# backtato/ai-video-detector

Hardware: AMD Instinct MI355X
Metric: sampled frames/sec analysed (1080p30 60 s clip, 2 fps sampling) (higher is better)
Workload: dtype u8 pixels; f32/f64 Farneback (cv2's own types); 1 GPU; BASELINE.json configs[1]: 1080p30 60 s clip, 2 fps sampling, one clip per GPU per step; frames_per_clip=120, height=1080, width=1920, clips_in_flight_per_gpu=3, fb_mode=fast+rerun, fb_wide160=2, parallelism=single GPU, rccl_ranks_seen=1

## Files before the change

ai-video-detector_amd/csrc/avd_farneback.hip:

```cpp
#include "avd_internal.h"
#include "avd_fb_device.h"

#pragma clang fp contract(off)

namespace {

constexpr int S = AVD_SMALL;

template <int K>
struct PyrGeo {
    static constexpr int WL = S >> K;
    static constexpr int NC = K == 0 ? S : 2 * WL;
    static constexpr int OFF = K == 0 ? 0 : (1 << K) / 2 - 1;
    static constexpr int TR = K >= 2 ? 4 : 8;
    static constexpr int STEPS = K >= 2 ? 2 : 1, BAND = STEPS * TR;
    static constexpr int TILES = WL / BAND;
    static constexpr int KS = K == 3 ? 19 : (K == 2 ? 9 : 3), HALF = KS / 2;
    static constexpr int SROWS = K == 0 ? TR + 2 * HALF : ((TR - 1) << K) + 2 + 2 * HALF;
    static constexpr int NEW = K == 0 ? TR : TR << K, KEEP = SROWS - NEW;
    static constexpr int PADX = 12, PS = S + 2 * PADX;
    static constexpr int SRC_BYTES = SROWS * PS, LDS_BYTES = SRC_BYTES + SROWS * NC * 4;
    static constexpr int FILTERED_PCT = TILES * (SROWS + (STEPS - 1) * NEW) * 100 / S;
    static_assert(WL % BAND == 0 && (K == 0 || FILTERED_PCT <= 120), "whole bands; a source row is filtered at most 1.2 times per frame");
    static_assert(STEPS == 1 || (KEEP * NC <= 4 * 256 && SRC_BYTES % 16 == 0 && (NEW * NC) % 4 == 0 && (KEEP * NC) % 4 == 0),
                  "the rows a step takes over move as one 16-byte piece per lane");
};
constexpr int cmax(int a, int b) { return a > b ? a : b; }
constexpr int cgcd(int a, int b) { return b == 0 ? a : cgcd(b, a % b); }

template <int PR>
struct PyrWalk {
    static constexpr int PER = PR / cgcd(256, PR), SG = 256 / cgcd(256, PR);
    __device__ static __forceinline__ void first(int tid, int& r, int& c)
    {
        r = 0; c = tid;
#pragma unroll
        for (int q = 1; q * PR < 256; q++)
            if (tid >= q * PR) { r = q; c = tid - q * PR; }
    }
    __device__ static __forceinline__ void next(int& r, int& c)
    {
        r += 256 / PR; c += 256 % PR;
        if (c >= PR) { c -= PR; r++; }
    }
};
constexpr int kPyrLds = cmax(cmax(PyrGeo<3>::LDS_BYTES, PyrGeo<2>::LDS_BYTES), cmax(PyrGeo<1>::LDS_BYTES, PyrGeo<0>::LDS_BYTES));

typedef float pyr_f4 __attribute__((ext_vector_type(4)));
typedef float pyr_f2 __attribute__((ext_vector_type(2)));

template <bool MA>
__device__ __forceinline__ float pyr_mac(float a, float b, float c)
{
    if constexpr (MA) return __fadd_rn(__fmul_rn(a, b), c);
    else return __builtin_fmaf(a, b, c);
}

template <int K, bool MA = false, bool LERP = false>
__device__ __forceinline__ void pyramid_step(char* lds, const uint8_t* __restrict__ img, const float (&kw)[PyrGeo<K>::KS], float* __restrict__ out,
                                             int y_first, int rb, pyr_f4& kept, bool more, int* __restrict__ diffword)
{
    using G = PyrGeo<K>;
    constexpr int WL = G::WL, NC = G::NC, OFF = G::OFF, TR = G::TR, KS = G::KS, HALF = G::HALF, SROWS = G::SROWS;
    constexpr int PADX = G::PADX, PS = G::PS;
    uint8_t (*src)[PS] = reinterpret_cast<uint8_t (*)[PS]>(lds);
    float (*rowf)[NC] = reinterpret_cast<float (*)[NC]>(lds + G::SRC_BYTES);
    const int tid = threadIdx.x;
    const bool cmp = K == 1 && diffword != nullptr;
    static_assert(K != 1 || G::STEPS == 1, "the pair-identity word is formed by a tile that loads all its source rows in one step");
    static_assert(HALF + 1 < S, "a source row is reflected at most once");
    auto row_at = [&](int r) -> unsigned { const int y = y_first + r; return (unsigned)(y < 0 ? -y : (y >= S ? 2 * S - 2 - y : y)) * S; };
    constexpr int NLD = (SROWS * (S / 4) + 255) / 256, NBD = (SROWS * 2 * HALF + 255) / 256;
    const int nld = (SROWS - rb) * (S / 4), nbd = (SROWS - rb) * 2 * HALF;
    constexpr int NBATCH = 8;
    int differs = 0;
#pragma unroll
    for (int e0 = 0; e0 < NLD; e0 += NBATCH) {
        const bool last = e0 + NBATCH >= NLD;
        unsigned v[NBATCH], vn[K == 1 ? NBATCH : 1];
        uint8_t bv[NBD];
#pragma unroll
        for (int e = e0; e < NLD && e < e0 + NBATCH; e++) {
            const int it = tid + 256 * e, q = it / (S / 4), c4 = it - q * (S / 4);
            if (it >= nld) continue;
            const unsigned at = row_at(rb + q) + 4u * c4;
            v[e - e0] = *reinterpret_cast<const unsigned*>(img + at);
            if (K == 1 && cmp) vn[e - e0] = *reinterpret_cast<const unsigned*>(img + (at + AVD_NPIX));
        }
#pragma unroll
        for (int e = 0; e < NBD; e++) {
            const int it = tid + 256 * e, q = it / (2 * HALF), i = it - q * (2 * HALF);
            if (!last || it >= nbd) continue;
            bv[e] = img[row_at(rb + q) + (unsigned)(i < HALF ? 1 + i : S - 2 - (i - HALF))];
        }
#pragma unroll
        for (int e = e0; e < NLD && e < e0 + NBATCH; e++) {
            const int it = tid + 256 * e, q = it / (S / 4), c4 = it - q * (S / 4);
            if (it >= nld) continue;
            reinterpret_cast<unsigned*>(src[rb + q] + PADX)[c4] = v[e - e0];
            if (K == 1 && cmp) differs |= v[e - e0] != vn[e - e0];
        }
#pragma unroll
        for (int e = 0; e < NBD; e++) {
            const int it = tid + 256 * e, q = it / (2 * HALF), i = it - q * (2 * HALF);
            if (!last || it >= nbd) continue;
            src[rb + q][i < HALF ? PADX - 1 - i : PADX + S + (i - HALF)] = bv[e];
        }
        __builtin_amdgcn_sched_barrier(0);
    }
    if (K == 1 && cmp) {
        const int any = __syncthreads_or(differs);
        if (tid == 0) *diffword = any;
    } else
        __syncthreads();
    if (G::STEPS > 1 && rb && tid < G::KEEP * NC / 4) reinterpret_cast<pyr_f4*>(&rowf[0][0])[tid] = kept;
    if (KS == 3) {
        static_assert(KS != 3 || NC == S, "the 3-tap scales filter whole rows");
        using W = PyrWalk<S / 4>;
        const unsigned* wp0[W::PER]; pyr_f4* dst0[W::PER]; int r0[W::PER];
        {
            int r, c4;
            W::first(tid, r, c4);
#pragma unroll
            for (int i = 0; i < W::PER; i++) {
                r0[i] = r;
                wp0[i] = reinterpret_cast<const unsigned*>(src[r] + PADX + 4 * c4);
                dst0[i] = reinterpret_cast<pyr_f4*>(&rowf[r][4 * c4]);
                W::next(r, c4);
            }
        }
        for (int sb = rb; sb < SROWS; sb += W::SG) {
#pragma unroll
            for (int i = 0; i < W::PER; i++) {
                if (256 * i >= SROWS * (S / 4) || r0[i] + sb >= SROWS) continue;
                const unsigned* wp = wp0[i] + sb * (PS / 4);
                const unsigned pw = wp[-1], cwd = wp[0], nw = wp[1];
                const float b[6] = {(float)(pw >> 24), (float)(cwd & 0xFFu), (float)((cwd >> 8) & 0xFFu), (float)((cwd >> 16) & 0xFFu),
                                    (float)(cwd >> 24), (float)(nw & 0xFFu)};
                pyr_f4 o;
#pragma unroll
                for (int e = 0; e < 4; e++) o[e] = pyr_mac<MA>(b[e + 1], kw[1], (b[e] + b[e + 2]) * kw[0]);
                dst0[i][sb * (NC / 4)] = o;
            }
        }
    } else {
        static_assert(KS == 3 || (K >= 2 && NC == 2 * WL), "the long filters run at the decimated scales, where the columns are pairs");
        using W = PyrWalk<WL>;
        constexpr int B0 = PADX + OFF - HALF, SH = B0 & 3, NW = (SH + KS + 1 + 3) / 4;
        const unsigned* wp0[W::PER]; pyr_f2* dst0[W::PER]; int r0[W::PER];
        {
            int r, jp;
            W::first(tid, r, jp);
#pragma unroll
            for (int i = 0; i < W::PER; i++) {
                r0[i] = r;
                wp0[i] = reinterpret_cast<const unsigned*>(src[r] + (B0 & ~3) + (jp << K));
                dst0[i] = reinterpret_cast<pyr_f2*>(&rowf[r][2 * jp]);
                W::next(r, jp);
            }
        }
        for (int sb = rb; sb < SROWS; sb += W::SG) {
#pragma unroll
            for (int i = 0; i < W::PER; i++) {
                if (256 * i >= SROWS * WL || r0[i] + sb >= SROWS) continue;
                const unsigned* wp = wp0[i] + sb * (PS / 4);
                unsigned d[NW];
#pragma unroll
                for (int q = 0; q < NW; q++) d[q] = wp[q];
                float b[KS + 1];
#pragma unroll
                for (int q = 0; q <= KS; q++) b[q] = (float)((d[(SH + q) >> 2] >> (8 * ((SH + q) & 3))) & 0xFFu);
                float v0 = 0.f, v1 = 0.f;
#pragma unroll
                for (int q = 0; q < KS; q++) {
                    v0 = pyr_mac<MA>(b[q], kw[q], v0);
                    v1 = pyr_mac<MA>(b[q + 1], kw[q], v1);
                }
                dst0[i][sb * (NC / 2)] = pyr_f2{v0, v1};
            }
        }
    }
    __syncthreads();
    auto colf = [&](const float* c) {
        float sacc = pyr_mac<MA>(c[0], kw[HALF], 0.f);
#pragma unroll
        for (int k = 1; k <= HALF; k++) sacc = pyr_mac<MA>(c[k * NC] + c[-k * NC], kw[HALF + k], sacc);
        return sacc;
    };
    {
        using W = PyrWalk<WL>;
        int dyl, dx;
        W::first(tid, dyl, dx);
#pragma unroll
        for (int i = 0; i < W::PER; i++) {
            if (256 * i < TR * WL) {
                for (int y = dyl; y < TR; y += W::SG) {
                    float o;
                    if (K == 0) {
                        o = colf(&rowf[y + HALF][dx]);
                    } else {
                        const pyr_f2* c = reinterpret_cast<const pyr_f2*>(&rowf[y << K][2 * dx]);
                        float w[2][2 * HALF + 2];
#pragma unroll
                        for (int q = 0; q < 2 * HALF + 2; q++) {
                            const pyr_f2 v = c[q * (NC / 2)];
                            w[0][q] = v.x; w[1][q] = v.y;
                        }
                        float p[2][2];
#pragma unroll
                        for (int a = 0; a < 2; a++)
#pragma unroll
                            for (int e = 0; e < 2; e++) {
                                float sacc = pyr_mac<MA>(w[e][HALF + a], kw[HALF], 0.f);
#pragma unroll
                                for (int k = 1; k <= HALF; k++) sacc = pyr_mac<MA>(w[e][HALF + a + k] + w[e][HALF + a - k], kw[HALF + k], sacc);
                                p[a][e] = sacc;
                            }
                        if constexpr (LERP && K >= 2) {
                            const float h0 = p[0][0] + (p[0][1] - p[0][0]) * 0.5f, h1 = p[1][0] + (p[1][1] - p[1][0]) * 0.5f;
                            o = h0 + (h1 - h0) * 0.5f;
                        } else
                            o = ((p[0][0] + p[0][1]) + (p[1][0] + p[1][1])) * 0.25f;
                    }
                    out[y * WL + dx] = o;
                }
            }
            W::next(dyl, dx);
        }
    }
    if (G::STEPS > 1 && more && tid < G::KEEP * NC / 4) kept = reinterpret_cast<const pyr_f4*>(&rowf[G::NEW][0])[tid];
}

template <int K, bool MA = false, bool LERP = false>
__device__ __forceinline__ void pyramid_body(char* lds, int blk, const uint8_t* __restrict__ small, const FbConsts* __restrict__ C,
                                             float* __restrict__ I, int n = 0, int* __restrict__ pairdiff = nullptr)
{
    using G = PyrGeo<K>;
    constexpr int WL = G::WL;
    const int f = blk / G::TILES, t = blk - f * G::TILES;
    const int dy0 = t * G::BAND;
    const uint8_t* img = small + (int64_t)f * AVD_NPIX;
    float* out = I + ((int64_t)f * WL + dy0) * WL;
    int* diffword = K == 1 && pairdiff != nullptr && f + 1 < n ? pairdiff + blk : nullptr;
    float kw[G::KS];
#pragma unroll
    for (int q = 0; q < G::KS; q++) kw[q] = C->gk[K][q];
    const int y_first = (K == 0 ? dy0 : (dy0 << K) + G::OFF) - G::HALF;
    pyr_f4 kept = {0.f, 0.f, 0.f, 0.f};
    for (int step = 0; step < G::STEPS; step++)
        pyramid_step<K, MA, LERP>(lds, img, kw, out + step * G::TR * WL, y_first + step * G::NEW, step ? G::KEEP : 0, kept, step + 1 < G::STEPS, diffword);
}


template <bool MA, bool LERP>
__device__ __forceinline__ void pyramid_all(char* lds, const uint8_t* __restrict__ small, int n, const FbConsts* __restrict__ C,
                                            float* __restrict__ I0, float* __restrict__ I1, float* __restrict__ I2,
                                            float* __restrict__ I3, int* __restrict__ flags, int* __restrict__ pairdiff)
{
    static_assert(PyrGeo<1>::TILES == kPairDiffTiles, "avd_fbfast.hip reads one word per 160-px tile");
    if (flags && (int)(blockIdx.x * 256 + threadIdx.x) < n - 1) flags[blockIdx.x * 256 + threadIdx.x] = 0;
    const int n3 = n * PyrGeo<3>::TILES, n2 = n * PyrGeo<2>::TILES, n1 = n * PyrGeo<1>::TILES;
    int b = blockIdx.x;
    if (b < n3) { pyramid_body<3, MA, LERP>(lds, b, small, C, I3); return; }
    b -= n3;
    if (b < n2) { pyramid_body<2, MA, LERP>(lds, b, small, C, I2); return; }
    b -= n2;
    if (b < n1) { pyramid_body<1, MA, LERP>(lds, b, small, C, I1, n, pairdiff); return; }
    if (I0) pyramid_body<0, MA, LERP>(lds, b - n1, small, C, I0);
}

__global__ __launch_bounds__(256) void k_pyramid_all(const uint8_t* __restrict__ small, int n, const FbConsts* __restrict__ C,
                                                    float* __restrict__ I0, float* __restrict__ I1, float* __restrict__ I2,
                                                    float* __restrict__ I3, int* __restrict__ flags, int* __restrict__ pairdiff)
{
    __shared__ __align__(16) char lds[kPyrLds];
    pyramid_all<false, false>(lds, small, n, C, I0, I1, I2, I3, flags, pairdiff);
}

template <bool MA, bool LERP>
__global__ __launch_bounds__(256) void k_pyramid_model(const uint8_t* __restrict__ small, int n, const FbConsts* __restrict__ C,
                                                      float* __restrict__ I0, float* __restrict__ I1, float* __restrict__ I2,
                                                      float* __restrict__ I3, int* __restrict__ flags, int* __restrict__ pairdiff)
{
    __shared__ __align__(16) char lds[kPyrLds];
    pyramid_all<MA, LERP>(lds, small, n, C, I0, I1, I2, I3, flags, pairdiff);
}

struct PolyPtrs { const float* I[AVD_FB_LEVELS]; float* R[AVD_FB_LEVELS]; const uint8_t* small; };

constexpr int kPolyRows = 16;
constexpr int kPolyQuads = 4 * (S / 4 + 10);
static_assert(AVD_FB_LEVELS == 4, "three walking scales and the one-row form of the coarsest");
__host__ __device__ constexpr int poly_wgs(int k) { return k < AVD_FB_LEVELS - 1 ? (S >> k) / kPolyRows : S >> (2 * k); }

typedef float pf4 __attribute__((ext_vector_type(4)));
typedef float pf2 __attribute__((ext_vector_type(2)));

__device__ __forceinline__ void polyexp_put(pf4* __restrict__ rowq, int x, int w, float t0, float t1, float t2)
{
    const pf4 t = {t0, t1, t1, t2};
    rowq[x + 5] = t;
    if (x == 0)
        for (int q = 0; q < 5; q++) rowq[q] = t;
    if (x == w - 1)
        for (int q = 0; q < 5; q++) rowq[w + 5 + q] = t;
}

__device__ __forceinline__ void polyexp_hpass(const pf4* __restrict__ rq, const float (&g)[6], const float (&xg)[6], const double (&gd)[6],
                                              const double (&xxgd)[6], double ig11, double ig03, double ig33, double ig55, float* __restrict__ o)
{
    const pf4 c = rq[0];
    double b1 = (double)(c.x * g[0]), b2 = 0, b3 = (double)(c.y * g[0]), b4 = 0, b5 = (double)(c.w * g[0]), b6 = 0;
#pragma unroll
    for (int q = 1; q <= 5; q++) {
        const pf4 p = rq[q], m = rq[-q];
        const pf2 s01 = p.xy + m.xy, d01 = p.xy - m.xy, s12 = p.zw + m.zw;
        const pf2 dx = d01 * pf2{xg[q], xg[q]};
        const pf2 sg = s12 * pf2{g[q], g[q]};
        const double tg = (double)s01.x;
        b1 = __builtin_fma(tg, gd[q], b1);
        b4 = __builtin_fma(tg, xxgd[q], b4);
        b2 += (double)dx.x;
        b3 += (double)sg.x;
        b6 += (double)dx.y;
        b5 += (double)sg.y;
    }
    o[0] = (float)(b3 * ig11);
    o[1] = (float)(b2 * ig11);
    o[2] = (float)(b1 * ig03 + b5 * ig33);
    o[3] = (float)(b1 * ig03 + b4 * ig33);
    o[4] = (float)(b6 * ig55);
}

template <int K, bool FOLD>
__device__ __forceinline__ void polyexp_rows(const float* __restrict__ img, const uint8_t* __restrict__ small, float* __restrict__ out, int y0,
                                             const FbConsts* __restrict__ C, pf4 (*rowb)[kPolyQuads], float (*outb)[S * 5])
{
    static_assert(!FOLD || K == 0, "only the 320-px scale forms its own blur");
    constexpr int w = S >> K, h = w, R = 1 << K, STEPS = kPolyRows / R;
    static_assert(R * (w + 10) <= kPolyQuads && h % kPolyRows == 0 && kPolyRows % R == 0, "a step's R rows fit one LDS buffer; whole bands");
    const int tid = threadIdx.x;
    const int sr = K == 0 ? 0 : tid / w, x = tid - sr * w;
    const int yb = y0 + sr;
    const int xs = x - 1 < 0 ? 0 : (x - 1 > w - 4 ? w - 4 : x - 1);
    const int shl = ((x == 0 ? 1 : x - 1) - xs) * 8, shc = (x - xs) * 8, shr = ((x == w - 1 ? w - 2 : x + 1) - xs) * 8;
    const float kx0 = C->gk[0][0], kx1 = C->gk[0][1], kx2 = C->gk[0][2];
    struct __attribute__((packed, aligned(1))) U4 { unsigned v; };
    auto hb = [&](int srow) __attribute__((always_inline)) {
        const int sr = srow < 0 ? -srow : (srow > h - 1 ? 2 * (h - 1) - srow : srow);
        const unsigned wd = reinterpret_cast<const U4*>(small + sr * w + xs)->v;
        const float l = (float)((wd >> shl) & 0xFFu), c = (float)((wd >> shc) & 0xFFu), r = (float)((wd >> shr) & 0xFFu);
        return __builtin_fmaf(c, kx1, (l + r) * kx0);
    };
    float hm = 0.f, h0 = 0.f, hp = 0.f;
    int rcur = -1000;
    auto blurred = [&](int r) __attribute__((always_inline)) {
        if (r != rcur) {
            if (r == rcur + 1) { hm = h0; h0 = hp; hp = hb(r + 1); }
            else { hm = hb(r - 1); h0 = hb(r); hp = hb(r + 1); }
            rcur = r;
        }
        return __builtin_fmaf(hp + hm, kx2, __builtin_fmaf(h0, kx1, 0.f));
    };
    auto pixel = [&](int r) __attribute__((always_inline)) { return FOLD ? blurred(r) : img[r * w + x]; };
    typedef float f4 __attribute__((ext_vector_type(4)));
    typedef float f2 __attribute__((ext_vector_type(2)));
    float g[6], xg[6], xxg[6];
    double gd[6], xxgd[6];
#pragma unroll
    for (int q = 0; q <= 5; q++) { g[q] = C->g[5 + q]; xg[q] = C->xg[5 + q]; xxg[q] = C->xxg[5 + q]; gd[q] = C->gd[q]; xxgd[q] = C->xxgd[q]; }
    const double ig11 = C->ig11, ig03 = C->ig03, ig33 = C->ig33, ig55 = C->ig55;
    float win[11 + kPolyRows - R];
#pragma unroll
    for (int q = 0; q < 10; q++) win[q] = pixel(min(max(yb - 5 + q, 0), h - 1));
    pf4* rowq[2] = {rowb[0] + sr * (w + 10), rowb[1] + sr * (w + 10)};
#pragma unroll
    for (int i = 0; i < STEPS; i++) {
        const int par = i & 1, o = R * i;
#pragma unroll
        for (int j = o + 11 - R; j <= o + 10; j++)
            if (j >= 10) win[j] = pixel(min(yb - 5 + j, h - 1));
        {
            f2 t02 = f2{win[o + 5] * g[0], 0.f};
            float t1 = 0.f;
#pragma unroll
            for (int q = 1; q <= 5; q++) {
                const float a = win[o + 5 - q], bb = win[o + 5 + q];
                const float p = a + bb;
                t02 = t02 + f2{g[q], xxg[q]} * f2{p, p};
                t1 = t1 + xg[q] * (bb - a);
            }
            polyexp_put(rowq[par], x, w, t02.x, t1, t02.y);
        }
        __syncthreads();
        if (i > 0) {
            f4* dst = reinterpret_cast<f4*>(out + (int64_t)(y0 + o - R) * w * 5);
            const f4* srcv = reinterpret_cast<const f4*>(outb[par ^ 1]);
            __builtin_nontemporal_store(srcv[tid], dst + tid);
            if (tid < S * 5 / 4 - 320) __builtin_nontemporal_store(srcv[tid + 320], dst + tid + 320);
        }
        polyexp_hpass(rowq[par] + x + 5, g, xg, gd, xxgd, ig11, ig03, ig33, ig55, outb[par] + tid * 5);
    }
    __syncthreads();
    {
        f4* dst = reinterpret_cast<f4*>(out + (int64_t)(y0 + kPolyRows - R) * w * 5);
        const f4* srcv = reinterpret_cast<const f4*>(outb[(STEPS - 1) & 1]);
        __builtin_nontemporal_store(srcv[tid], dst + tid);
        if (tid < S * 5 / 4 - 320) __builtin_nontemporal_store(srcv[tid + 320], dst + tid + 320);
    }
}

__global__ __launch_bounds__(320) void k_polyexp_all(PolyPtrs P, int n, const FbConsts* __restrict__ C)
{
    __shared__ pf4 rowb[2][kPolyQuads];
    __shared__ __align__(16) float outbb[2][S * 5];
    pf4* row = rowb[0];
    static_assert(8 * (S / 8 + 10) <= 2 * kPolyQuads, "the eight sub-rows of the coarsest scale fit");
    float* outb = outbb[0];
    int b = (int)blockIdx.x, k = 0, wgs = 0;
    for (; k < AVD_FB_LEVELS; k++) {
        wgs = n * poly_wgs(k);
        const int cnt = ((wgs + 7) >> 3) << 3;
        if (b < cnt) break;
        b -= cnt;
    }
    if (k >= AVD_FB_LEVELS) return;
    const int per = (wgs + 7) >> 3, lid = (b & 7) * per + (b >> 3);
    if (lid >= wgs) return;
    const int w = S >> k, h = w;
    int f = 0;
#pragma unroll
    for (int kk = 0; kk < AVD_FB_LEVELS; kk++)
        if (k == kk) f = lid / poly_wgs(kk);
    const int t = lid - f * poly_wgs(k);
    float* R = P.R[k] + (int64_t)f * w * h * 5;
    if (k == 0) {
        if (P.small) polyexp_rows<0, true>(nullptr, P.small + (int64_t)f * S * S, R, t * kPolyRows, C, rowb, outbb);
        else polyexp_rows<0, false>(P.I[0] + (int64_t)f * S * S, nullptr, R, t * kPolyRows, C, rowb, outbb);
        return;
    }
    if (k == 1) { polyexp_rows<1, false>(P.I[1] + (int64_t)f * w * h, nullptr, R, t * kPolyRows, C, rowb, outbb); return; }
    if (k == 2) { polyexp_rows<2, false>(P.I[2] + (int64_t)f * w * h, nullptr, R, t * kPolyRows, C, rowb, outbb); return; }
    const int y0 = t << k;
    const int tid = threadIdx.x;
    const int sr = tid / w, x = tid - sr * w;
    const int y = y0 + sr;
    const float* img = P.I[k] + (int64_t)f * w * h;
    float g[6], xg[6], xxg[6];
    double gd[6], xxgd[6];
#pragma unroll
    for (int q = 0; q <= 5; q++) { g[q] = C->g[5 + q]; xg[q] = C->xg[5 + q]; xxg[q] = C->xxg[5 + q]; gd[q] = C->gd[q]; xxgd[q] = C->xxgd[q]; }
    pf4* rowq = row + sr * (w + 10);
    {
        float t0 = img[y * w + x] * g[0], t1 = 0.f, t2 = 0.f;
#pragma unroll
        for (int q = 1; q <= 5; q++) {
            const float a = img[max(y - q, 0) * w + x], bb = img[min(y + q, h - 1) * w + x];
            const float p = a + bb;
            t0 = t0 + g[q] * p;
            t1 = t1 + xg[q] * (bb - a);
            t2 = t2 + xxg[q] * p;
        }
        polyexp_put(rowq, x, w, t0, t1, t2);
    }
    __syncthreads();
    polyexp_hpass(rowq + x + 5, g, xg, gd, xxgd, C->ig11, C->ig03, C->ig33, C->ig55, outb + tid * 5);
    __syncthreads();
    typedef float f4 __attribute__((ext_vector_type(4)));
    f4* dst = reinterpret_cast<f4*>(R + (int64_t)y0 * w * 5);
    const f4* srcv = reinterpret_cast<const f4*>(outb);
    __builtin_nontemporal_store(srcv[tid], dst + tid);
    if (tid < S * 5 / 4 - 320) __builtin_nontemporal_store(srcv[tid + 320], dst + tid + 320);
}

template <int W, bool LERP = false>
__global__ __launch_bounds__(256) void k_flow_up(const float* __restrict__ prev, float* __restrict__ flow, int npairs, const int* __restrict__ plist)
{
    constexpr int H = W, PW = W / 2, PH = H / 2, Q = W / 4;
    const int gid = blockIdx.x * 256 + threadIdx.x;
    if (gid >= npairs * 2 * H * Q) return;
    const int q = gid % Q;
    const int dy = (gid / Q) % H;
    int pc = gid / (Q * H);
    if (plist) pc = plist[pc >> 1] * 2 + (pc & 1);
    const float* src = prev + (int64_t)pc * PW * PH;
    float fy = dy * 0.5f - 0.25f;
    const int sy = floor_f(fy);
    fy -= sy;
    const float* r0 = src + clampi(sy, 0, PH - 1) * PW;
    const float* r1 = src + clampi(sy + 1, 0, PH - 1) * PW;
    const float b0 = 1.f - fy, b1 = fy;
    float o[4];
#pragma unroll
    for (int i = 0; i < 4; i++) {
        const int dx = q * 4 + i;
        float fx = dx * 0.5f - 0.25f;
        int sx = floor_f(fx);
        fx -= sx;
        if (sx < 0) { fx = 0; sx = 0; }
        bool edge = false;
        if (sx + 1 >= PW) { edge = true; if (sx >= PW - 1) { fx = 0; sx = PW - 1; } }
        const int x1 = min(sx + 1, PW - 1);
        const float a0 = 1.f - fx, a1 = fx;
        float d0, d1;
        if (edge) { d0 = r0[sx] * 1.f; d1 = r1[sx] * 1.f; }
        else if constexpr (LERP) { d0 = r0[sx] + (r0[x1] - r0[sx]) * a1; d1 = r1[sx] + (r1[x1] - r1[sx]) * a1; }
        else { d0 = r0[sx] * a0 + r0[x1] * a1; d1 = r1[sx] * a0 + r1[x1] * a1; }
        if constexpr (LERP) o[i] = (d0 + (d1 - d0) * b1) * 2.f;
        else o[i] = (d0 * b0 + d1 * b1) * 2.f;
    }
    *reinterpret_cast<float4*>(flow + ((int64_t)pc * H + dy) * W + q * 4) = make_float4(o[0], o[1], o[2], o[3]);
}

constexpr int kChunk = 8192;
constexpr int kNChunk = (AVD_NPIX + kChunk - 1) / kChunk;

__device__ __forceinline__ float chunk_total(const float* part)
{
    float t = part[0];
#pragma unroll
    for (int i = 1; i < kNChunk; i++) t += part[i];
    return t;
}

__global__ __launch_bounds__(512) void k_stats_pair(const float* __restrict__ mag, float* __restrict__ stats, const int* __restrict__ plist)
{
    __shared__ float wpart[kNChunk][8];
    __shared__ float ctot[kNChunk];
    const int p = plist ? plist[blockIdx.x] : (int)blockIdx.x, tid = threadIdx.x;
    const int l = tid >> 3, wave = tid >> 6;
    const bool in_last = l < ((AVD_NPIX - (kNChunk - 1) * kChunk) >> 7);
    const float* src = mag + (int64_t)p * AVD_NPIX + l * 128 + (tid & 7);
    float v[kNChunk][16];
#pragma unroll
    for (int c = 0; c < kNChunk; c++)
#pragma unroll
        for (int k = 0; k < 16; k++) v[c][k] = (c < kNChunk - 1 || in_last) ? src[c * kChunk + 8 * k] : 0.f;
    float total[2];
#pragma unroll
    for (int pass = 0; pass < 2; pass++) {
#pragma unroll
        for (int c = 0; c < kNChunk; c++) {
            float r = v[c][0];
#pragma unroll
            for (int k = 1; k < 16; k++) r += v[c][k];
#pragma unroll
            for (int d = 1; d < 64; d <<= 1) r = r + __shfl_down(r, d);
            if ((tid & 63) == 0) wpart[c][wave] = r;
        }
        __syncthreads();
        if (tid < kNChunk) {
            const float* w = wpart[tid];
            ctot[tid] = tid < kNChunk - 1 ? ((w[0] + w[1]) + (w[2] + w[3])) + ((w[4] + w[5]) + (w[6] + w[7])) : (w[0] + w[1]) + (w[2] + w[3]);
        }
        __syncthreads();
        total[pass] = chunk_total(ctot);
        if (pass == 0) {
            const float mean32 = total[0] / (float)AVD_NPIX;
#pragma unroll
            for (int c = 0; c < kNChunk; c++)
#pragma unroll
                for (int k = 0; k < 16; k++) { const float d = v[c][k] - mean32; v[c][k] = d * d; }
            __syncthreads();
        }
    }
    if (tid == 0) {
        stats[2 * p] = (float)((double)total[0] / (double)AVD_NPIX);
        stats[2 * p + 1] = (float)((double)total[1] / (double)AVD_NPIX);
    }
}

__global__ void k_mag(const float* __restrict__ flow, float* __restrict__ mag, int64_t total4, const int* __restrict__ plist)
{
    const int64_t gid = (int64_t)blockIdx.x * 256 + threadIdx.x;
    if (gid >= total4) return;
    const int64_t ps = gid / (AVD_NPIX / 4), i = gid - ps * (AVD_NPIX / 4);
    const int64_t p = plist ? plist[ps] : ps;
    const float4 fx = reinterpret_cast<const float4*>(flow + p * 2 * AVD_NPIX)[i], fy = reinterpret_cast<const float4*>(flow + (p * 2 + 1) * AVD_NPIX)[i];
    float4 m;
    m.x = sqrtf(fx.x * fx.x + fy.x * fy.x);
    m.y = sqrtf(fx.y * fx.y + fy.y * fy.y);
    m.z = sqrtf(fx.z * fx.z + fy.z * fy.z);
    m.w = sqrtf(fx.w * fx.w + fy.w * fy.w);
    reinterpret_cast<float4*>(mag + p * AVD_NPIX)[i] = m;
}

__global__ void k_flow_interleave(const float* __restrict__ flow, float* __restrict__ out, int64_t total)
{
    const int64_t gid = (int64_t)blockIdx.x * 256 + threadIdx.x;
    if (gid >= total) return;
    const int64_t p = gid / AVD_NPIX, i = gid - p * AVD_NPIX;
    out[gid * 2] = flow[p * 2 * AVD_NPIX + i];
    out[gid * 2 + 1] = flow[(p * 2 + 1) * AVD_NPIX + i];
}

template <typename... A>
inline void launch1d(void (*k)(A...), int64_t items, int block, hipStream_t s, A... args)
{
    const int grid = (int)((items + block - 1) / block);
    if (grid > 0) hipLaunchKernelGGL(k, dim3(grid), dim3(block), 0, s, args...);
}

constexpr int kLevelId[AVD_FB_LEVELS] = {AVD_K_LEVEL320, AVD_K_LEVEL160, AVD_K_LEVEL80, AVD_K_LEVEL40};
constexpr int kFlowUpId[AVD_FB_LEVELS - 1] = {AVD_K_FLOWUP320, AVD_K_FLOWUP160, AVD_K_FLOWUP80};

void pyramid_and_polyexp(avd_ctx* ctx, const FlowCall& call, const uint8_t* d_small, int n)
{
    Workspace& ws = ctx->ws;
    const FbConsts* C = ctx->d_fbc;
    const bool fold = fb_fold_blur_eff(ctx->fb_fold_blur, call.model) != 0;
    const int wgs = n * ((fold ? 0 : PyrGeo<0>::TILES) + PyrGeo<1>::TILES + PyrGeo<2>::TILES + PyrGeo<3>::TILES);
    kmark(ctx, AVD_K_PYRAMID);
    auto pyramid = [&](auto kernel) {
        hipLaunchKernelGGL(kernel, dim3(wgs), dim3(256), 0, ctx->stream, d_small, n, C, fold ? nullptr : ws.d_pyr[0].p, ws.d_pyr[1].p, ws.d_pyr[2].p,
                           ws.d_pyr[3].p, ws.d_fbflags.p, ws.d_pairdiff.p);
    };
    switch (call.model & (kCv2GaussMuladd | kCv2ResizeLerp)) {
    case 0: pyramid(k_pyramid_all); break;
    case kCv2GaussMuladd: pyramid(k_pyramid_model<true, false>); break;
    case kCv2ResizeLerp: pyramid(k_pyramid_model<false, true>); break;
    default: pyramid(k_pyramid_model<true, true>); break;
    }
    PolyPtrs P;
    P.small = fold ? d_small : nullptr;
    int grid = 0;
    for (int k = 0; k < AVD_FB_LEVELS; k++) {
        P.I[k] = ws.d_pyr[k]; P.R[k] = ws.d_poly[k];
        grid += ((n * poly_wgs(k) + 7) >> 3) << 3;
    }
    kmark(ctx, AVD_K_POLYEXP);
    hipLaunchKernelGGL(k_polyexp_all, dim3(grid), dim3(320), 0, ctx->stream, P, n, C);
}

void flow_up_level(hipStream_t stream, int k, const float* prev, float* flow, int np, const int* plist, bool lerp)
{
    fb_dispatch_width(S >> k, [&](auto wc) {
        constexpr int W = decltype(wc)::value;
        if constexpr (W > S / 8) {
            if (lerp) launch1d(k_flow_up<W, true>, (int64_t)np * 2 * W * (W / 4), 256, stream, prev, flow, np, plist);
            else launch1d(k_flow_up<W>, (int64_t)np * 2 * W * (W / 4), 256, stream, prev, flow, np, plist);
        }
    });
}

int exact_levels(avd_ctx* ctx, const FlowCall& call, int np, int fused_mask, FbTwoScratch scratch, const int* plist, FbChunk& chunk)
{
    const int top = fb_coarsest(call.model);
    const bool lerp = (call.model & kCv2ResizeLerp) != 0;
    Workspace& ws = ctx->ws;
    const hipStream_t stream = ctx->stream;
    const bool rerun = plist != nullptr;
    float* const flow0 = rerun ? const_cast<float*>(chunk.flow[0]) : ws.d_flow[0].p;
    if (rerun) kmark(ctx, AVD_K_RERUN);
    for (int k = top; k >= 0; k--) {
        const int w = S >> k;
        const bool coarsest = k == top, fused = (fused_mask >> k) & 1;
        float* flow = k == 0 ? flow0 : ws.d_flow[k].p;
        if (coarsest) {
            if (!fused && rerun) { ctx->err = "exact re-run: the coarsest level runs the fused kernel (it needs no cleared flow)"; return AVD_ERR_ARG; }
            if (!fused) HIP_TRY(ctx, hipMemsetAsync(flow, 0, sizeof(float) * 2 * w * w * np, stream));
        } else {
            if (!rerun) kmark(ctx, kFlowUpId[k]);
            flow_up_level(stream, k, ws.d_flow[k + 1], flow, np, plist, lerp);
        }
        if (!rerun) { chunk.flow[k] = flow; kmark(ctx, kLevelId[k]); }
        const bool marks = !rerun && k == 0;
        if (fused) {
            level320_mark(ctx, marks);
            if (int e = launch_fb_level(ctx, stream, w, ws.d_poly[k], flow, np, 3, coarsest, plist)) return e;
            level320_mark(ctx, marks);
        } else {
            for (int it = 0; it < 3; it++)
                if (int e = launch_fb_two(ctx, stream, w, ws.d_poly[k], flow, scratch, np, plist, marks)) return e;
        }
    }
    return 0;
}

int fast_levels(avd_ctx* ctx, const FlowCall& call, int np, FbChunk& chunk)
{
    Workspace& ws = ctx->ws;
    const hipStream_t stream = ctx->stream;
    const int fold = fb_fold_up_eff(ctx->fb_fold_up, call.model), top = fb_coarsest(call.model);
    const bool fold160 = fb_fold_up160_eff(ctx->fb_fold_up160, call.model) != 0, lerp = (call.model & kCv2ResizeLerp) != 0;
    int* flags = ctx->fb_rerun ? ws.d_fbflags.p : nullptr;
    const int* pairdiff = ctx->fb_rerun ? ws.d_pairdiff.p : nullptr;
    for (int k = top; k >= 0; k--) {
        const int w = S >> k;
        const bool coarsest = k == top, three = (k == 2 || k == 3) && (fold & 4);
        float *a = ws.d_flow[k], *b = ws.d_flow2[k];
        const float* prev = coarsest ? nullptr : chunk.flow[k + 1];
        const bool chain = (k == 0 && (fold & 1)) || (k == 1 && fold160 && call.wide160);
        const bool cleared = coarsest && k != AVD_FB_LEVELS - 1;
        static_assert(2 * (S >> (AVD_FB_LEVELS - 2)) * (S >> (AVD_FB_LEVELS - 2)) >= kPairDiffTiles, "the cleared flow serves as the identity words");
        if (cleared) HIP_TRY(ctx, hipMemsetAsync(a, 0, sizeof(float) * 2 * w * w * np, stream));
        const FbFlowFrom from = cleared ? FbFlowFrom::level : coarsest ? FbFlowFrom::zero : chain ? FbFlowFrom::chain
                                : ((k == 1 || k == 2) && (fold & 2)) ? FbFlowFrom::prologue : FbFlowFrom::level;
        if (from == FbFlowFrom::level && !coarsest) {
            kmark(ctx, kFlowUpId[k]);
            flow_up_level(stream, k, prev, a, np, nullptr, lerp);
        }
        const bool from_prev = from == FbFlowFrom::chain || from == FbFlowFrom::prologue;
        kmark(ctx, kLevelId[k]);
        level320_mark(ctx, k == 0);
        if (three) {
            const FbFastLaunch L{call.wide160, 3, from, from_prev ? prev : a, b, a, nullptr, flags, pairdiff};
            if (int e = launch_fb_fast(ctx, stream, w, ws.d_poly[k], L, np)) return e;
            a = b;
        } else {
            for (int it = 0; it < 3; it++) {
                float* mag = (k == 0 && it == 2) ? ws.d_mag.p : nullptr;
                const int* identity = cleared && it == 0 && pairdiff ? reinterpret_cast<const int*>(a) : pairdiff;
                const FbFastLaunch L{call.wide160, 1, it == 0 ? from : FbFlowFrom::level, it == 0 && from_prev ? prev : a, b, a, mag, flags, identity};
                if (int e = launch_fb_fast(ctx, stream, w, ws.d_poly[k], L, np)) return e;
                float* t = a; a = b; b = t;
            }
        }
        level320_mark(ctx, k == 0);
        chunk.flow[k] = a;
    }
    return 0;
}

void flow_tail(avd_ctx* ctx, const FlowCall& call, const float* flow, bool with_mag, int m, const int* plist, int np_chunk)
{
    Workspace& ws = ctx->ws;
    const hipStream_t stream = ctx->stream;
    if (with_mag) launch1d(k_mag, (int64_t)m * (AVD_NPIX / 4), 256, stream, flow, ws.d_mag.p, (int64_t)m * (AVD_NPIX / 4), plist);
    hipLaunchKernelGGL(k_stats_pair, dim3(m), dim3(512), 0, stream, (const float*)ws.d_mag, ws.d_stats.p, plist);
    if (call.dense_flow && ws.d_flow_il)
        launch1d(k_flow_interleave, (int64_t)np_chunk * AVD_NPIX, 256, stream, flow, ws.d_flow_il.p, (int64_t)np_chunk * AVD_NPIX);
}

}

int launch_farneback(avd_ctx* ctx, const FlowCall& call, const uint8_t* d_small, int n, FbChunk* left)
{
    if (n < 2) return 0;
    Workspace& ws = ctx->ws;
    if (ctx->profiling) ctx->kern_ev_used = 0;
    const bool fast = ctx->fb_mode == 1;
    FbChunk& chunk = ws.fb_holds;
    chunk.mag_valid = fast;
    pyramid_and_polyexp(ctx, call, d_small, n);
    if (int e = fast ? fast_levels(ctx, call, n - 1, chunk) : exact_levels(ctx, call, n - 1, ctx->fb_fused, {ws.d_vs, ws.d_vs0}, nullptr, chunk)) return e;
    HIP_TRY(ctx, hipGetLastError());
    *left = chunk;
    return 0;
}

int launch_farneback_rerun(avd_ctx* ctx, const FlowCall& call, const int* h_list, int m, int np_chunk)
{
    if (m <= 0) return 0;
    Workspace& ws = ctx->ws;
    if (m > ws.fb_cap) { ctx->err = "re-run list longer than the chunk"; return AVD_ERR_ARG; }
    if (int e = ws.d_rlist.reserve(ctx, (size_t)ws.fb_cap)) return e;
    const int fused_mask = m <= kRerunTwoKernelMax ? ((ctx->fb_rerun_fused & 0xF) | (1 << fb_coarsest(call.model))) : 0xF;
    if (fused_mask != 0xF) {
        const FbTwoScratchSize sz = fb_two_scratch_size(kRerunTwoKernelMax);
        if (int e = ws.d_vs0_rerun.reserve(ctx, sz.vs0)) return e;
        if (int e = ws.d_vs_rerun.reserve(ctx, sz.vs)) return e;
    }
    HIP_TRY(ctx, hipMemcpyAsync(ws.d_rlist, h_list, sizeof(int) * m, hipMemcpyHostToDevice, ctx->stream));
    if (int e = exact_levels(ctx, call, m, fused_mask, {ws.d_vs_rerun, ws.d_vs0_rerun}, ws.d_rlist, ws.fb_holds)) return e;
    flow_tail(ctx, call, ws.fb_holds.flow[0], true, m, ws.d_rlist, np_chunk);
    HIP_TRY(ctx, hipGetLastError());
    return 0;
}

int launch_flow_stats(avd_ctx* ctx, const FlowCall& call, const FbChunk& chunk, int n)
{
    if (n < 2) return 0;
    kmark(ctx, AVD_K_STATS);
    flow_tail(ctx, call, chunk.flow[0], !chunk.mag_valid, n - 1, nullptr, n - 1);
    HIP_TRY(ctx, hipGetLastError());
    return 0;
}
```

Measured before the change: 143,600 frames/s.

## Prefetch next polyexp source rows one step ahead via a compile-time row plan

Replaces the runtime row-cache bookkeeping (rcur compare, branches, per-row reflect/clamp) in the polyexp row walk with a constexpr slot plan. The next step's source rows are issued right after the barrier, so the global load overlaps the output store and the horizontal pass. For the folded 320-px scale, it also keeps a sliding array of horizontally filtered rows instead of recomputing them. Edge clamping becomes selects that copy the neighbouring slot. This raises register use (hs, srcq, rowq_ arrays) and depends on the plan header matching the kernel constants.

Result: no change. 144,800 frames/s, median of 6 (+0.8%).

```diff
diff --git a/ai-video-detector_amd/csrc/avd_farneback.hip b/ai-video-detector_amd/csrc/avd_farneback.hip
--- a/ai-video-detector_amd/csrc/avd_farneback.hip
+++ b/ai-video-detector_amd/csrc/avd_farneback.hip
@@ -1,5 +1,6 @@
 #include "avd_internal.h"
 #include "avd_fb_device.h"
+#include "avd_polyexp_plan.h"
 
 #pragma clang fp contract(off)
 
@@ -341,28 +342,22 @@
     static_assert(R * (w + 10) <= kPolyQuads && h % kPolyRows == 0 && kPolyRows % R == 0, "a step's R rows fit one LDS buffer; whole bands");
     const int tid = threadIdx.x;
     const int sr = K == 0 ? 0 : tid / w, x = tid - sr * w;
-    const int yb = y0 + sr;
+    namespace pp = avd_polyplan;
+    static_assert(pp::kSide == S && pp::kBandRows == kPolyRows && pp::side(K) == h && pp::step_rows(K) == R && pp::steps(K) == STEPS, "one plan");
     const int xs = x - 1 < 0 ? 0 : (x - 1 > w - 4 ? w - 4 : x - 1);
     const int shl = ((x == 0 ? 1 : x - 1) - xs) * 8, shc = (x - xs) * 8, shr = ((x == w - 1 ? w - 2 : x + 1) - xs) * 8;
     const float kx0 = C->gk[0][0], kx1 = C->gk[0][1], kx2 = C->gk[0][2];
     struct __attribute__((packed, aligned(1))) U4 { unsigned v; };
-    auto hb = [&](int srow) __attribute__((always_inline)) {
-        const int sr = srow < 0 ? -srow : (srow > h - 1 ? 2 * (h - 1) - srow : srow);
-        const unsigned wd = reinterpret_cast<const U4*>(small + sr * w + xs)->v;
+    auto src_word = [&](int m) __attribute__((always_inline)) {
+        return reinterpret_cast<const U4*>(small + pp::src_row(y0, m) * w + xs)->v;
+    };
+    auto hfilt = [&](unsigned wd) __attribute__((always_inline)) {
         const float l = (float)((wd >> shl) & 0xFFu), c = (float)((wd >> shc) & 0xFFu), r = (float)((wd >> shr) & 0xFFu);
         return __builtin_fmaf(c, kx1, (l + r) * kx0);
     };
-    float hm = 0.f, h0 = 0.f, hp = 0.f;
-    int rcur = -1000;
-    auto blurred = [&](int r) __attribute__((always_inline)) {
-        if (r != rcur) {
-            if (r == rcur + 1) { hm = h0; h0 = hp; hp = hb(r + 1); }
-            else { hm = hb(r - 1); h0 = hb(r); hp = hb(r + 1); }
-            rcur = r;
-        }
+    auto blur = [&](float hm, float h0, float hp) __attribute__((always_inline)) {
         return __builtin_fmaf(hp + hm, kx2, __builtin_fmaf(h0, kx1, 0.f));
     };
-    auto pixel = [&](int r) __attribute__((always_inline)) { return FOLD ? blurred(r) : img[r * w + x]; };
     typedef float f4 __attribute__((ext_vector_type(4)));
     typedef float f2 __attribute__((ext_vector_type(2)));
     float g[6], xg[6], xxg[6];
@@ -370,16 +365,52 @@
 #pragma unroll
     for (int q = 0; q <= 5; q++) { g[q] = C->g[5 + q]; xg[q] = C->xg[5 + q]; xxg[q] = C->xxg[5 + q]; gd[q] = C->gd[q]; xxgd[q] = C->xxgd[q]; }
     const double ig11 = C->ig11, ig03 = C->ig03, ig33 = C->ig33, ig55 = C->ig55;
-    float win[11 + kPolyRows - R];
-#pragma unroll
-    for (int q = 0; q < 10; q++) win[q] = pixel(min(max(yb - 5 + q, 0), h - 1));
+    float win[pp::slots(K)];
+    float hs[FOLD ? pp::src_slots() : 1];
+    unsigned srcq[STEPS];
+    float rowq_[STEPS][R];
+    auto fetch = [&](int i) __attribute__((always_inline)) {
+        if constexpr (FOLD) srcq[i] = src_word(pp::src_first_slot(i));
+        else {
+#pragma unroll
+            for (int q = 0; q < R; q++) rowq_[i][q] = img[pp::slot_row(K, y0, sr, pp::first_slot(K, i) + q) * w + x];
+        }
+    };
+    auto take = [&](int i) __attribute__((always_inline)) {
+        if constexpr (FOLD) {
+            const int j = pp::first_slot(0, i);
+            hs[j + 2] = hfilt(srcq[i]);
+            const float v = blur(hs[j], hs[j + 1], hs[j + 2]);
+            const float prev = win[j - 1];
+            win[j] = pp::slot_may_be_below(0, j) && pp::slot_below(0, y0, 0, j) ? prev : v;
+        } else {
+#pragma unroll
+            for (int q = 0; q < R; q++) win[pp::first_slot(K, i) + q] = rowq_[i][q];
+        }
+    };
+    if constexpr (FOLD) {
+        unsigned wd[pp::src_slot_count(0)];
+#pragma unroll
+        for (int m = 0; m < pp::src_slot_count(0); m++) wd[m] = src_word(m);
+#pragma unroll
+        for (int m = 0; m < pp::src_slot_count(0); m++) hs[m] = hfilt(wd[m]);
+#pragma unroll
+        for (int j = 0; j < pp::kTaps; j++) win[j] = blur(hs[j], hs[j + 1], hs[j + 2]);
+#pragma unroll
+        for (int j = pp::kHalf - 1; j >= 0; j--)
+        {
+            const float own = win[j], next = win[j + 1];
+            win[j] = pp::slot_above(y0, 0, j) ? next : own;
+        }
+    } else {
+#pragma unroll
+        for (int j = 0; j < pp::kTaps; j++) win[j] = img[pp::slot_row(K, y0, sr, j) * w + x];
+    }
     pf4* rowq[2] = {rowb[0] + sr * (w + 10), rowb[1] + sr * (w + 10)};
 #pragma unroll
     for (int i = 0; i < STEPS; i++) {
         const int par = i & 1, o = R * i;
-#pragma unroll
-        for (int j = o + 11 - R; j <= o + 10; j++)
-            if (j >= 10) win[j] = pixel(min(yb - 5 + j, h - 1));
+        if (i > 0) take(i);
         {
             f2 t02 = f2{win[o + 5] * g[0], 0.f};
             float t1 = 0.f;
@@ -393,6 +424,7 @@
             polyexp_put(rowq[par], x, w, t02.x, t1, t02.y);
         }
         __syncthreads();
+        if (pp::ahead_count(K, i) > 0) fetch(i + 1);
         if (i > 0) {
             f4* dst = reinterpret_cast<f4*>(out + (int64_t)(y0 + o - R) * w * 5);
             const f4* srcv = reinterpret_cast<const f4*>(outb[par ^ 1]);
diff --git a/ai-video-detector_amd/csrc/avd_polyexp_plan.h b/ai-video-detector_amd/csrc/avd_polyexp_plan.h
--- /dev/null
+++ b/ai-video-detector_amd/csrc/avd_polyexp_plan.h
@@ -0,0 +1,47 @@
+#pragma once
+
+#if defined(__HIPCC__)
+#define AVD_POLYPLAN_FN __host__ __device__ constexpr
+#else
+#define AVD_POLYPLAN_FN constexpr
+#endif
+
+namespace avd_polyplan {
+
+constexpr int kSide = 320;
+constexpr int kBandRows = 16;
+constexpr int kWalkScales = 3;
+constexpr int kTaps = 11, kHalf = 5;
+
+AVD_POLYPLAN_FN int side(int k) { return kSide >> k; }
+AVD_POLYPLAN_FN int step_rows(int k) { return 1 << k; }
+AVD_POLYPLAN_FN int steps(int k) { return kBandRows >> k; }
+AVD_POLYPLAN_FN int bands(int k) { return side(k) / kBandRows; }
+AVD_POLYPLAN_FN int slots(int k) { return kTaps + kBandRows - step_rows(k); }
+
+AVD_POLYPLAN_FN int clamp(int v, int lo, int hi) { return v < lo ? lo : (v > hi ? hi : v); }
+AVD_POLYPLAN_FN int reflect101(int r, int h) { return r < 0 ? -r : (r > h - 1 ? 2 * (h - 1) - r : r); }
+
+AVD_POLYPLAN_FN int slot_unclamped(int y0, int sr, int j) { return y0 + sr - kHalf + j; }
+AVD_POLYPLAN_FN int slot_row(int k, int y0, int sr, int j) { return clamp(slot_unclamped(y0, sr, j), 0, side(k) - 1); }
+AVD_POLYPLAN_FN bool slot_above(int y0, int sr, int j) { return slot_unclamped(y0, sr, j) < 0; }
+AVD_POLYPLAN_FN bool slot_below(int k, int y0, int sr, int j) { return slot_unclamped(y0, sr, j) > side(k) - 1; }
+AVD_POLYPLAN_FN bool slot_fresh(int k, int y0, int sr, int j) { return !slot_above(y0, sr, j) && !slot_below(k, y0, sr, j); }
+AVD_POLYPLAN_FN bool slot_may_be_above(int j) { return j < kHalf; }
+AVD_POLYPLAN_FN bool slot_may_be_below(int k, int j) { return j > kBandRows + kHalf - step_rows(k); }
+
+AVD_POLYPLAN_FN int first_slot(int k, int i) { return i == 0 ? 0 : step_rows(k) * i + kTaps - step_rows(k); }
+AVD_POLYPLAN_FN int slot_count(int k, int i) { return i == 0 ? kTaps : step_rows(k); }
+AVD_POLYPLAN_FN int ahead_count(int k, int i) { return i + 1 < steps(k) ? slot_count(k, i + 1) : 0; }
+AVD_POLYPLAN_FN int ahead_first_slot(int k, int i) { return first_slot(k, i + 1); }
+
+AVD_POLYPLAN_FN int src_slots() { return slots(0) + 2; }
+AVD_POLYPLAN_FN bool src_needed(int y0, int m) { return y0 - 6 + m >= -1 && y0 - 6 + m <= kSide; }
+AVD_POLYPLAN_FN int src_row(int y0, int m) { return reflect101(clamp(y0 - 6 + m, -1, kSide), kSide); }
+AVD_POLYPLAN_FN int blur_src_row(int y0, int j, int d) { return reflect101(slot_row(0, y0, 0, j) + d, kSide); }
+AVD_POLYPLAN_FN int src_first_slot(int i) { return i == 0 ? 0 : first_slot(0, i) + 2; }
+AVD_POLYPLAN_FN int src_slot_count(int i) { return i == 0 ? kTaps + 2 : 1; }
+AVD_POLYPLAN_FN int src_ahead_count(int i) { return i + 1 < steps(0) ? src_slot_count(i + 1) : 0; }
+AVD_POLYPLAN_FN int src_ahead_first_slot(int i) { return src_first_slot(i + 1); }
+
+}
```
